# knight46/Quantum_compute_DFT

Hardware: AMD Instinct MI355X
Metric: grid_points_per_sec (higher is better)
Workload: dtype f64; 1 GPU; benzene_gga_def2svp: DFT_ComputeXC (GGA) nao=114 ngrid=143556 per GPU, synthetic AO/grid (SURVEY 8(d) recipe), inputs resident in HBM; functional=GGA, nao=114, nocc=21, ngrid_per_gpu=143556, entry_point=DFT_ComputeXC (the reference ABI: full density matrix)

## Files before the change

### include/dft_solver.h

```cpp
#ifndef QCDFT_AMD_DFT_SOLVER_H
#define QCDFT_AMD_DFT_SOLVER_H

#ifdef __cplusplus
extern "C" {
#endif

typedef struct XCSolver XCSolver;

enum SolverType { SOLVER_LDA = 0, SOLVER_GGA = 1, SOLVER_B3LYP = 2,
                  SOLVER_MIX = 3  };

enum XCComponent { XC_SLATER_X = 0, XC_VWN5_C, XC_VWN_RPA_C, XC_PW92_C,
                   XC_PBE_X, XC_PBE_C, XC_B88_X, XC_LYP_C, XC_NCOMP };


XCSolver *DFT_CreateSolver(int type);

void DFT_DestroySolver(XCSolver *solver);

double DFT_ComputeXC(XCSolver *solver, int ngrid, int nao,
                     unsigned long long d_dm_ptr,
                     unsigned long long d_ao_ptr,
                     unsigned long long d_ao_grad_ptr,
                     unsigned long long d_weights_ptr,
// ... 149 lines not shown
int DFT_ComputeXCGradient(XCSolver *solver, long long ngrid, int nao, unsigned long long d_dm_ptr,
                          unsigned long long d_ao_ptr, unsigned long long d_weights_ptr, unsigned long long d_ao_grad_ptr,
                          unsigned long long d_ao_hess_ptr, unsigned long long d_out_ptr);
int DFT_ComputeXCGradientSpin(XCSolver *solver, long long ngrid, int nao, unsigned long long d_dm_a_ptr,
                              unsigned long long d_dm_b_ptr, unsigned long long d_ao_ptr, unsigned long long d_weights_ptr,
                              unsigned long long d_ao_grad_ptr, unsigned long long d_ao_hess_ptr,
                              unsigned long long d_out_ptr);

int DFT_ComputeXCGradientMeta(XCSolver *solver, long long ngrid, int nao, unsigned long long d_dm_ptr,
                              unsigned long long d_ao_ptr, unsigned long long d_weights_ptr,
                              unsigned long long d_ao_grad_ptr, unsigned long long d_ao_hess_ptr,
                              unsigned long long d_out_ptr);
int DFT_ComputeXCEnergyDensityMeta(XCSolver *solver, long long ngrid, int nao, unsigned long long d_dm_ptr,
                                   unsigned long long d_ao_ptr, unsigned long long d_ao_grad_ptr,
                                   unsigned long long d_e_out_ptr);

int DFT_ComputeXCEnergyDensity(XCSolver *solver, long long ngrid, int nao, unsigned long long d_dm_ptr,
                               unsigned long long d_ao_ptr, unsigned long long d_ao_grad_ptr, unsigned long long d_e_out_ptr);
int DFT_ComputeXCEnergyDensitySpin(XCSolver *solver, long long ngrid, int nao, unsigned long long d_dm_a_ptr,
                                   unsigned long long d_dm_b_ptr, unsigned long long d_ao_ptr, unsigned long long d_ao_grad_ptr,
                                   unsigned long long d_e_out_ptr);
int DFT_BeckeWeightGradient(XCSolver *solver, long long ngrid, int natm, const double *atom_xyz, const double *atom_radius,
                            unsigned long long d_coords_ptr, unsigned long long d_owner_ptr, unsigned long long d_f_ptr,
                            unsigned long long d_cell_out_ptr, unsigned long long d_out_ptr);

void *DFT_EriColumnsOpen(int nshell, const double *shl_xyz, const int *shl_l, const int *shl_nprim,
                         const int *shl_off, const int *shl_ao, const double *prim_exp, const double *prim_coef,
                         int nao, int nprim_total, const double *qmax_pairs);
int DFT_EriColumns(void *handle, int shell_C, int shell_D, double screen, unsigned long long d_out_ptr);
int DFT_EriColumnsMany(void *handle, int npairs, const int *shell_C, const int *shell_D, double screen,
                       unsigned long long d_out_ptr, const long long *offsets);
int DFT_EriColumnsSetStream(void *handle, unsigned long long hip_stream);
const char *DFT_EriColumnsLastError(void *handle);
void DFT_EriColumnsClose(void *handle);

void *DFT_PointCoulombOpen(int nshell, const double *shl_xyz, const int *shl_l, const int *shl_nprim,
                           const int *shl_off, const int *shl_ao, const double *prim_exp, const double *prim_coef,
                           int nao, int nprim_total);
int DFT_PointCoulombMatrix(void *handle, long long npts, unsigned long long d_points_xyz, unsigned long long d_weights,
                           unsigned long long d_out);
int DFT_PointCoulombContract(void *handle, long long npts, unsigned long long d_points_xyz, unsigned long long d_dm,
                             unsigned long long d_out);
int DFT_PointCoulombField(void *handle, long long npts, unsigned long long d_points_xyz, unsigned long long d_dm,
                          unsigned long long d_out);
int DFT_PointCoulombSetStream(void *handle, unsigned long long hip_stream);
const char *DFT_PointCoulombLastError(void *handle);
void DFT_PointCoulombClose(void *handle);

void *DFT_Grad2eOpen(int nshell, const double *shl_xyz, const int *shl_l, const int *shl_nprim, const int *shl_off,
                     const int *shl_ao, const double *prim_exp, const double *prim_coef, int nao, int nprim_total);
int DFT_Grad2e(void *handle, unsigned long long d_dm, double c_hf, unsigned long long d_out);
int DFT_Grad2eSpin(void *handle, unsigned long long d_dm, unsigned long long d_ms, double c_hf, unsigned long long d_out);
int DFT_Grad2eSetStream(void *handle, unsigned long long hip_stream);
const char *DFT_Grad2eLastError(void *handle);
void DFT_Grad2eClose(void *handle);

void *DFT_ScfTailOpen(int nao, int nocc, unsigned long long d_hcore, unsigned long long d_overlap, unsigned long long d_basis,
                      unsigned long long d_fock_out, unsigned long long d_mo_energy);
int DFT_ScfTailSetStream(void *handle, unsigned long long hip_stream);
int DFT_ScfTailStep(void *handle, int rotate, double c_hf, double tol, double canon_tol, int max_inner, int slot, int nhist,
                    const int *hist, const double *coef, unsigned long long d_J, unsigned long long d_K,
                    unsigned long long d_vraw, unsigned long long d_dm, unsigned long long d_cocc, unsigned long long d_exc);
int DFT_ScfTailFinish(void *handle, double c_hf, unsigned long long d_J, unsigned long long d_K, unsigned long long d_dm,
                      unsigned long long d_cocc);
int DFT_ScfTailMore(void *handle, int nsteps, unsigned long long d_J, unsigned long long d_K, unsigned long long d_dm,
                    unsigned long long d_cocc, unsigned long long d_exc);
int DFT_ScfTailSetStepsHint(void *handle, int nsteps);
int DFT_ScfTailWait(void *handle, double *out8);
int DFT_ScfTailGram(void *handle, double *host_out64);
int DFT_ScfTailStamps(void *handle, long long *host_out16);
const char *DFT_ScfTailLastError(void *handle);
void DFT_ScfTailClose(void *handle);

int DFT_SetOption(XCSolver *solver, const char *key, double value);

double DFT_GetOption(XCSolver *solver, const char *key);

int DFT_SetStream(XCSolver *solver, unsigned long long hip_stream);

const char *DFT_GetLastError(XCSolver *solver);

int DFT_GetTimings(XCSolver *solver, double *ms, const char **names, int max_entries);

#ifdef __cplusplus
}
#endif
#endif
```

### quantum_compute_dft_amd/csrc/dft_api.hip

```cpp
#include <hip/hip_runtime.h>

#include <cmath>
#include <cstdarg>
#include <cstdio>
#include <cstdint>
#include <cstdlib>
#include <cstring>
#include <algorithm>
#include <limits>
#include <string>
#include <type_traits>
#include <vector>

#include "../../include/dft_solver.h"
#include "ao_kernels.hpp"
#include "jk_kernels.hpp"
#include "cd_kernels.hpp"
#include "cd_response_kernels.hpp"
#include "xc_big_kernels.hpp"
#include "xc_ws_kernels.hpp"
#include "xc_kernels.hpp"
#include "xc_occ_launch.hpp"
#include "xc_tiny_launch.hpp"
#include "dm_factor_launch.hpp"
// ... 2302 lines not shown
    }
    if (!strcmp(key, "eri_symmetric")) { s->eri_sym = value == 2.0 ? 2 : value != 0.0; return 0; }
    if (!strcmp(key, "graph")) { s->graph = value > 0.0 ? 1 : value < 0.0 ? -1 : 0; return 0; }
    if (!strcmp(key, "quirks")) { s->quirks = value != 0.0; s->fxc[0].ngrid = 0; return 0; }
    if (!strcmp(key, "path")) { s->path = (int)value; return 0; }
    if (!strcmp(key, "profile")) { s->profile = value != 0.0; return 0; }
    if (!strcmp(key, "spin_wait")) { s->spin_wait = value != 0.0; return 0; }
    if (!strcmp(key, "strict_sync")) { s->strict_sync = value != 0.0; return 0; }
    if (!strcmp(key, "fuse_finish")) { s->fuse_finish = value != 0.0; return 0; }
    if (!strcmp(key, "vxc_fringe")) { s->vxc_fringe = value > 0.0 ? 1 : value < 0.0 ? -1 : 0; return 0; }
    if (!strcmp(key, "publish")) { s->publish = value > 0.0 ? 1 : value < 0.0 ? -1 : 0; return 0; }
    if (!strcmp(key, "sweep_order")) { s->sweep_order = (int)value & 3; return 0; }
    if (!strcmp(key, "occ")) { s->occ = value == 1.0 ? 1 : value == 2.0 ? 2 : 0; return 0; }
    if (!strcmp(key, "dm_factor")) { s->dm_factor = value != 0.0; return 0; }
    if (!strcmp(key, "tiny")) { s->tiny = value > 0.0 ? 1 : value < 0.0 ? -1 : 0; return 0; }
    if (!strcmp(key, "ao_pt")) { s->ao_pt = value == 16.0 ? 16 : value == 8.0 ? 8 : 0; return 0; }
    if (!strcmp(key, "ksplit")) { s->ksplit = value > 0 ? (int)value : 0; return 0; }
    if (!strcmp(key, "xcg_spin_fused")) { s->xcg_spin_fused = value != 0.0; return 0; }
    if (!strcmp(key, "meta_fused")) { s->meta_fused = value != 0.0; return 0; }
    if (!strcmp(key, "xcg_meta_fused")) { s->xcg_meta_fused = value != 0.0; return 0; }
    if (!strcmp(key, "tau_spin_fused")) { s->tau_spin_fused = value != 0.0; return 0; }
    return -1;
}

double DFT_GetOption(XCSolver *s, const char *key)
{
    const double unknown = std::numeric_limits<double>::quiet_NaN();
    if (!s || !key) return unknown;
    if (!strcmp(key, "publish")) return s->publish;
    if (!strcmp(key, "publish_probe")) return s->publish_ok ? 1.0 : 0.0;
    if (!strcmp(key, "publish_live")) return s->publish > 0 && s->publish_ok ? 1.0 : 0.0;
    if (!strcmp(key, "used_publish")) return s->used_publish;
    if (!strcmp(key, "vxc_fringe")) return s->vxc_fringe;
    if (!strcmp(key, "used_vxc_fringe")) return s->used_vxc_fringe;
    if (!strcmp(key, "fuse_finish")) return s->fuse_finish;
    if (!strcmp(key, "strict_sync")) return s->strict_sync;
    if (!strcmp(key, "spin_wait")) return s->spin_wait;
    if (!strcmp(key, "graph")) return s->graph;
    if (!strcmp(key, "tiny")) return s->tiny;
    if (!strcmp(key, "sweep_order")) return s->sweep_order;
    if (!strcmp(key, "path")) return s->path;
    if (!strcmp(key, "quirks")) return s->quirks;
    if (!strcmp(key, "occ")) return s->occ;
    if (!strcmp(key, "used_occ")) return s->used_occ;
    if (!strcmp(key, "dm_factor")) return s->dm_factor;
    if (!strcmp(key, "used_dm_factor")) return s->used_dm_factor;
    if (!strcmp(key, "xcg_spin_fused")) return s->xcg_spin_fused;
    if (!strcmp(key, "meta_fused")) return s->meta_fused;
    if (!strcmp(key, "xcg_meta_fused")) return s->xcg_meta_fused;
    if (!strcmp(key, "tau_spin_fused")) return s->tau_spin_fused;
    if (!strcmp(key, "dm_factor_rank")) return s->dm_factor_rank;
    return unknown;
}

int DFT_SetStream(XCSolver *s, unsigned long long hip_stream)
{
    if (!s) return -1;
    DeviceGuard dg(s);
    if (s->device_ok) (void)hipStreamSynchronize(s->stream);
    s->stream = (hipStream_t)hip_stream;
    return 0;
}

const char *DFT_GetLastError(XCSolver *s)
{
    return s ? s->last_error.c_str() : "";
}

int DFT_GetTimings(XCSolver *s, double *ms, const char **names, int max_entries)
{
    if (!s || !s->device_ok) return 0;
    DeviceGuard dg(s);
    (void)hipStreamSynchronize(s->stream);
    int n = 0;
    for (size_t i = 0; i < s->n_timed && n < max_entries; ++i, ++n) {
        float t = 0.f;
        if (hipEventElapsedTime(&t, s->timings[i].t0, s->timings[i].t1) != hipSuccess) t = -1.f;
        if (ms) ms[n] = t;
        if (names) names[n] = s->timings[i].name;
    }
    return n;
}

}
```

### quantum_compute_dft_amd/csrc/xc_ws_kernels.hpp

```cpp
#pragma once
#include <hip/hip_runtime.h>
#include "xc_kernels.hpp"

namespace qcdft {

#ifdef QCDFT_STAMPS
__device__ unsigned long long g_stamps[256 * 8 * 4];
#define QCDFT_T(var) unsigned long long var = __builtin_amdgcn_s_memtime()
#define QCDFT_ACC(slot, a, b) st_acc[slot] += (b) - (a)
#else
#define QCDFT_T(var)
#define QCDFT_ACC(slot, a, b)
#endif

constexpr int WS_ROWS = 16;
constexpr int WS_THREADS = 512;
constexpr int WS_RING = 4;
constexpr int WS_OT = 16;

template <int NT> struct WsCfg {
    static constexpr int NCOL = 16 * NT;
    static constexpr int JN = (NT + 1) / 2;
    static constexpr int LDA = NCOL + 2;
    static constexpr int LDX = ((NCOL + 31) / 32) * 32 + 16;
};

__device__ __forceinline__ unsigned ws_tile(unsigned ntile, unsigned b, unsigned s, unsigned nwg, int rev)
{
    const unsigned t = b + s * nwg;
    return rev ? ntile - 1u - t : t;
}

template <int NT, int FP>
__device__ __forceinline__ void vxc_ws_mfma_fringe(const double *Ps, const double *Qs, int tid, int wave, int nao, long nstep,
                                                   double *__restrict__ slab)
{
    using C = WsCfg<NT>;
    constexpr int NF = NT - 1, F0 = 16 * NF;
    constexpr int TILE = WS_ROWS * C::LDX;
    constexpr int NOPP = F0 + 4 > 64 ? 2 : 1;
    static_assert(NT >= 2 && F0 + 4 <= 128, "one whole tile at least, two opposite indices per lane at most");
    const int lane = tid & 63, li = lane & 15, lk = lane >> 4;
    constexpr bool FRW = FP > 0;
    constexpr int ROWS = FRW ? (NF > 6 ? 1 : 0) : 2, RA = ROWS ? ROWS : 1, NL = FRW ? 2 * FP : 1;
    const int nr = FRW || NF >= 6 ? ROWS : min(2, max(0, NF - 2 * wave));
    d4 acc[RA][NF];
#pragma unroll
    for (int i = 0; i < RA; ++i)
#pragma unroll
        for (int j = 0; j < NF; ++j) acc[i][j] = (d4){0.0, 0.0, 0.0, 0.0};
    double fa[NL][NOPP], fb[NL][NOPP];
#pragma unroll
    for (int f = 0; f < NL; ++f)
#pragma unroll
        for (int j = 0; j < NOPP; ++j) { fa[f][j] = 0.0; fb[f][j] = 0.0; }
    int opp[NOPP];
#pragma unroll
    for (int j = 0; j < NOPP; ++j) opp[j] = min(lane + 64 * j, C::NCOL - 1);

    const int fo = lk * C::LDX + li;
    double af[RA], bf[NF];
    auto load_frags = [&](int slot, int ks, double (&a_)[RA], double (&b_)[NF]) {
        if (ROWS == 0) return;
        const double *P = Ps + slot * TILE + fo + 4 * ks * C::LDX;
        const double *Q = Qs + slot * TILE + fo + 4 * ks * C::LDX;
#pragma unroll
        for (int i = 0; i < RA; ++i) a_[i] = Q[16 * min(2 * wave + i, NF - 1)];
#pragma unroll
        for (int j = 0; j < NF; ++j) b_[j] = P[16 * j];
    };
    auto fringe_pair = [&](const double *Pr, const double *Qr, const double (&po)[NOPP], const double (&qo)[NOPP], int f) {
        const double2 pf = *reinterpret_cast<const double2 *>(&Pr[F0 + f]);
        const double2 qf = *reinterpret_cast<const double2 *>(&Qr[F0 + f]);
#pragma unroll
        for (int j = 0; j < NOPP; ++j) {
            fa[f][j] += qf.x * po[j];
            fa[f + 1][j] += qf.y * po[j];
            fb[f][j] += qo[j] * pf.x;
            fb[f + 1][j] += qo[j] * pf.y;
        }
    };
#pragma unroll
    for (int i = 0; i < RA; ++i) af[i] = 0.0;
#pragma unroll
    for (int j = 0; j < NF; ++j) bf[j] = 0.0;
    for (long base = 0; base < nstep; base += WS_RING) {
#pragma unroll
        for (int u = 0; u < WS_RING; ++u) {
            const long step = base + u;
            if (step >= 2 && step < nstep) {
                if (step == 2) load_frags((u + 2) % WS_RING, 0, af, bf);
#pragma unroll
                for (int ks = 0; ks < WS_ROWS / 4; ++ks) {
                    double an[RA], bn[NF];
                    if (ks + 1 < WS_ROWS / 4) load_frags((u + 2) % WS_RING, ks + 1, an, bn);
                    else                      load_frags((u + 3) % WS_RING, 0, an, bn);
#pragma unroll
                    for (int i = 0; i < ROWS; ++i)
                        if (i < nr) {
#pragma unroll
                            for (int j = 0; j < NF; ++j) acc[i][j] = mfma_f64(af[i], bf[j], acc[i][j]);
                        }
                    if (FRW) {
#pragma unroll
                        for (int kk = 0; kk < 4; ++kk) {
                            const double *Pr = Ps + ((u + 2) % WS_RING) * TILE + (4 * ks + kk) * C::LDX;
                            const double *Qr = Qs + ((u + 2) % WS_RING) * TILE + (4 * ks + kk) * C::LDX;
                            double po[NOPP], qo[NOPP];
#pragma unroll
                            for (int j = 0; j < NOPP; ++j) { po[j] = Pr[opp[j]]; qo[j] = Qr[opp[j]]; }
                            fringe_pair(Pr, Qr, po, qo, 0);
                            if (FP > 1) fringe_pair(Pr, Qr, po, qo, 2);
                        }
                    }
#pragma unroll
                    for (int i = 0; i < RA; ++i) af[i] = an[i];
#pragma unroll
                    for (int j = 0; j < NF; ++j) bf[j] = bn[j];
                    __builtin_amdgcn_sched_barrier(0);
                }
            }
            __syncthreads();
        }
    }
#pragma unroll
    for (int i = 0; i < ROWS; ++i) {
        if (i >= nr) continue;
#pragma unroll
        for (int j = 0; j < NF; ++j)
#pragma unroll
            for (int r = 0; r < 4; ++r)
                slab[(size_t)(16 * (2 * wave + i) + lk + 4 * r) * nao + 16 * j + li] = acc[i][j][r];
    }
    if (FRW) {
#pragma unroll
        for (int f = 0; f < NL; ++f) {
            if (F0 + f >= nao) continue;
#pragma unroll
            for (int j = 0; j < NOPP; ++j) {
                const int o = lane + 64 * j;
                if (o < nao) slab[(size_t)(F0 + f) * nao + o] = fa[f][j];
                if (o < F0)  slab[(size_t)o * nao + F0 + f] = fb[f][j];
            }
        }
    }
}

template <int NT, bool GRAD, bool VEC, bool SYM, bool FR = false>
__global__ __launch_bounds__(WS_THREADS, 2) void k_vxc_ws(long ngrid, int nao,
                                                          const double *__restrict__ ao,
                                                          const double *__restrict__ gx,
                                                          const double *__restrict__ gy,
                                                          const double *__restrict__ gz,
                                                          const double *__restrict__ coef,
                                                          double *__restrict__ slabs, int rev)
{
    using C = WsCfg<NT>;
    constexpr int TILE = WS_ROWS * C::LDX;
    constexpr int NTW = (NT + 1) / 2;
    __shared__ double ring[2 * WS_RING * TILE];
    double *const Ps = ring, *const Qs = ring + WS_RING * TILE;

    const int tid = threadIdx.x;
    const int wave = __builtin_amdgcn_readfirstlane(tid >> 6);
    const long ntile = (ngrid + WS_ROWS - 1) / WS_ROWS;
    const long nloc = (ntile > (long)blockIdx.x) ? (ntile - blockIdx.x + gridDim.x - 1) / gridDim.x : 0;
    const long nstep = nloc + 2;

    if constexpr (FR) {
        static_assert(!FR || !SYM, "the fringe variant writes one-sided slabs");
        double *slab = slabs + (size_t)blockIdx.x * nao * nao;
        if (wave < 3)                                 vxc_ws_mfma_fringe<NT, 0>(Ps, Qs, tid, wave, nao, nstep, slab);
        else if (wave == 3 && nao - 16 * (NT - 1) <= 2) vxc_ws_mfma_fringe<NT, 1>(Ps, Qs, tid, 3, nao, nstep, slab);
        else if (wave == 3)                           vxc_ws_mfma_fringe<NT, 2>(Ps, Qs, tid, 3, nao, nstep, slab);
    }
    if (!FR && wave < 4) {
        const int lane = tid & 63, li = lane & 15, lk = lane >> 4;
        const int wa = wave >> 1, wb = wave & 1;
        const int na = (NT - wa + 1) / 2, nb = (NT - wb + 1) / 2;
        d4 acc[NTW][NTW];
#pragma unroll
        for (int i = 0; i < NTW; ++i)
#pragma unroll
            for (int j = 0; j < NTW; ++j) acc[i][j] = (d4){0.0, 0.0, 0.0, 0.0};

#ifdef QCDFT_STAMPS
        unsigned long long st_acc[4] = {0, 0, 0, 0};
#endif
        const int fo = lk * C::LDX + li;
        double af[NTW], bf[NTW];
        auto load_frags = [&](int slot, int ks, double (&a_)[NTW], double (&b_)[NTW]) {
            const double *P = Ps + slot * TILE + fo + 4 * ks * C::LDX;
            const double *Q = Qs + slot * TILE + fo + 4 * ks * C::LDX;
#pragma unroll
            for (int i = 0; i < NTW; ++i) {
                a_[i] = Q[16 * min(wa + 2 * i, NT - 1)];
                b_[i] = P[16 * min(wb + 2 * i, NT - 1)];
            }
        };
#pragma unroll
        for (int i = 0; i < NTW; ++i) { af[i] = 0.0; bf[i] = 0.0; }
        for (long base = 0; base < nstep; base += WS_RING) {
#pragma unroll
            for (int u = 0; u < WS_RING; ++u) {
                const long step = base + u;
                QCDFT_T(ta);
                if (step >= 2 && step < nstep) {
                    if (step == 2) load_frags((u + 2) % WS_RING, 0, af, bf);
#pragma unroll
                    for (int ks = 0; ks < WS_ROWS / 4; ++ks) {
                        double an[NTW], bn[NTW];
                        if (ks + 1 < WS_ROWS / 4) load_frags((u + 2) % WS_RING, ks + 1, an, bn);
                        else                      load_frags((u + 3) % WS_RING, 0, an, bn);
#pragma unroll
                        for (int i = 0; i < NTW; ++i)
#pragma unroll
                            for (int j = 0; j < NTW; ++j)
                                if ((2 * i + 1 < NT || i < na) && (2 * j + 1 < NT || j < nb))
                                    acc[i][j] = mfma_f64(af[i], bf[j], acc[i][j]);
#pragma unroll
                        for (int i = 0; i < NTW; ++i) { af[i] = an[i]; bf[i] = bn[i]; }
                    }
                }
                QCDFT_T(tb);
                __syncthreads();
                QCDFT_T(tc);
                QCDFT_ACC(0, ta, tb);
                QCDFT_ACC(1, tb, tc);
            }
        }
#ifdef QCDFT_STAMPS
        if ((tid & 63) == 0) { g_stamps[(blockIdx.x * 8 + wave) * 4 + 0] = st_acc[0]; g_stamps[(blockIdx.x * 8 + wave) * 4 + 1] = st_acc[1]; }
#endif
        double *slab = slabs + (size_t)blockIdx.x * nao * nao;
        if (!SYM) {
#pragma unroll
            for (int i = 0; i < NTW; ++i)
#pragma unroll
                for (int j = 0; j < NTW; ++j) {
                    if (i >= na || j >= nb) continue;
                    const int b = 16 * (wb + 2 * j) + li;
#pragma unroll
                    for (int r = 0; r < 4; ++r) {
                        const int a = 16 * (wa + 2 * i) + lk + 4 * r;
                        if (a < nao && b < nao) slab[(size_t)a * nao + b] = acc[i][j][r];
                    }
                }
        } else {
            constexpr int LDM = C::NCOL + 1;
            static_assert(LDM * C::NCOL <= 2 * WS_RING * TILE, "M tile must fit in the ring");
            double *M = ring;
#pragma unroll
            for (int i = 0; i < NTW; ++i)
#pragma unroll
                for (int j = 0; j < NTW; ++j) {
                    if (i >= na || j >= nb) continue;
                    const int b = 16 * (wb + 2 * j) + li;
#pragma unroll
                    for (int r = 0; r < 4; ++r) M[(16 * (wa + 2 * i) + lk + 4 * r) * LDM + b] = acc[i][j][r];
                }
        }
    } else if (wave >= 4) {
        __builtin_amdgcn_s_setprio(3);
        const int lt = tid - 256, row = lt >> 4, seg = lt & 15;
        const double *c0 = coef, *c1 = coef + (size_t)ngrid, *c2 = coef + 2 * (size_t)ngrid,
                     *c3 = coef + 3 * (size_t)ngrid;
        double p0[2][2 * C::JN], p1[2][2 * C::JN], p2[2][2 * C::JN], p3[2][2 * C::JN];
        double k0[2], k1[2], k2[2], k3[2];

        const long plane = ngrid * (long)nao;
        const unsigned voff = (unsigned)(row * nao + 2 * seg) * 8u, koff = (unsigned)row * 8u;
        const unsigned tile_b = (unsigned)(WS_ROWS * nao) * 8u, ktile_b = WS_ROWS * 8u;
        const unsigned plane_b = (unsigned)(plane * 8), coef_b = (unsigned)(ngrid * 8);
        const __amdgpu_buffer_rsrc_t r0 = plane_rsrc(ao, plane), r1 = plane_rsrc(GRAD ? gx : ao, plane),
                                     r2 = plane_rsrc(GRAD ? gy : ao, plane), r3 = plane_rsrc(GRAD ? gz : ao, plane),
                                     q0 = plane_rsrc(c0, ngrid), q1 = plane_rsrc(GRAD ? c1 : c0, ngrid),
                                     q2 = plane_rsrc(GRAD ? c2 : c0, ngrid), q3 = plane_rsrc(GRAD ? c3 : c0, ngrid);
        auto issue = [&](int set, unsigned s) {
            const bool live = s < (unsigned)nloc;
            const unsigned t = ws_tile((unsigned)ntile, blockIdx.x, s, gridDim.x, rev);
            const unsigned so = live ? t * tile_b : plane_b, ko = live ? t * ktile_b : coef_b;
            k0[set] = buf_load_f64(q0, koff, ko);
            if (GRAD) {
                k1[set] = buf_load_f64(q1, koff, ko);
                k2[set] = buf_load_f64(q2, koff, ko);
                k3[set] = buf_load_f64(q3, koff, ko);
            }
            buf_load_row<C::JN, VEC>(r0, voff, so, p0[set]);
            if (GRAD) {
                buf_load_row<C::JN, VEC>(r1, voff, so, p1[set]);
                buf_load_row<C::JN, VEC>(r2, voff, so, p2[set]);
                buf_load_row<C::JN, VEC>(r3, voff, so, p3[set]);
            }
        };
        issue(0, 0);
        __builtin_amdgcn_sched_barrier(0);
        issue(1, 1);
        __builtin_amdgcn_sched_barrier(0);
#ifdef QCDFT_STAMPS
        unsigned long long st_acc[4] = {0, 0, 0, 0};
#endif

        for (long base = 0; base < nstep; base += WS_RING) {
#pragma unroll
            for (int u = 0; u < WS_RING; ++u) {
                const long step = base + u;
                const int set = u & 1;
                QCDFT_T(ta);
#ifdef QCDFT_STAMPS
                asm volatile("s_waitcnt vmcnt(20)" ::: "memory");
#endif
                QCDFT_T(tw);
                {
                    double *P = Ps + u * TILE, *Q = Qs + u * TILE;
#pragma unroll
                    for (int j = 0; j < C::JN; ++j) {
                        const int c = 32 * j + 2 * seg;
                        if (c < C::NCOL) {
                            const double a0 = p0[set][2 * j], b0 = p0[set][2 * j + 1];
                            double qa = k0[set] * a0, qb = k0[set] * b0;
                            if (GRAD) {
                                qa += k1[set] * p1[set][2 * j] + k2[set] * p2[set][2 * j] + k3[set] * p3[set][2 * j];
                                qb += k1[set] * p1[set][2 * j + 1] + k2[set] * p2[set][2 * j + 1] + k3[set] * p3[set][2 * j + 1];
                            }
                            *reinterpret_cast<double2 *>(&Q[row * C::LDX + c]) = make_double2(qa, qb);
                            *reinterpret_cast<double2 *>(&P[row * C::LDX + c]) = make_double2(a0, b0);
                        }
                    }
                    QCDFT_T(tm);
                    issue(set, (unsigned)step + 2u);
                    QCDFT_ACC(3, tw, tm);
                }
                QCDFT_T(tb);
                __syncthreads();
                QCDFT_T(tc);
                QCDFT_ACC(0, ta, tw);
                QCDFT_ACC(1, tw, tb);
                QCDFT_ACC(2, tb, tc);
            }
        }
#ifdef QCDFT_STAMPS
        if ((tid & 63) == 0) { for (int q = 0; q < 4; ++q) g_stamps[(blockIdx.x * 8 + wave) * 4 + q] = st_acc[q]; }
#endif
    }
    if (SYM) {
        constexpr int LDM = C::NCOL + 1;
        const double *M = ring;
        __syncthreads();
        double *slab = slabs + (size_t)blockIdx.x * nao * nao;
        for (int e = tid; e < nao * nao; e += WS_THREADS) {
            const int a = e / nao, b = e - a * nao;
            slab[e] = M[a * LDM + b] + M[b * LDM + a];
        }
    }
}

template <int NT, bool GRAD, bool VEC>
__global__ __launch_bounds__(WS_THREADS, 2) void k_rho_ws(long ngrid, int nao,
                                                          const double *__restrict__ ao,
                                                          const double *__restrict__ gx,
                                                          const double *__restrict__ gy,
                                                          const double *__restrict__ gz,
                                                          const double *__restrict__ dm,
                                                          double *__restrict__ rho,
                                                          double *__restrict__ grad,
                                                          double *__restrict__ sigma, int rev)
{
    using C = WsCfg<NT>;
    constexpr int NKS = 4 * NT;
    constexpr int NTW = (NT + 3) / 4;
    constexpr int ATILE = WS_ROWS * C::LDA, XTILE = WS_ROWS * C::LDX;
    constexpr int NQ = GRAD ? 4 : 1;
    constexpr int LDS_ = WS_ROWS + 2, SQ = 320, STILE = NQ * SQ;
    static_assert(WS_ROWS * LDS_ <= SQ, "a partial-sum plane must fit its stride");
    __shared__ double As[WS_RING * ATILE];
    __shared__ double Xs[2 * XTILE];
    __shared__ double Ss[2 * STILE];
    __shared__ double Ob[(WS_OT + 1) * WS_ROWS * 4];

    const int tid = threadIdx.x;
    const int wave = __builtin_amdgcn_readfirstlane(tid >> 6);
    const unsigned ntile = (unsigned)((ngrid + WS_ROWS - 1) / WS_ROWS);
    const unsigned nwg = gridDim.x, wg = blockIdx.x;
    const unsigned nloc = ntile > wg ? (ntile - wg + nwg - 1) / nwg : 0u;
    const unsigned nstep = nloc + 3;

    if (wave < 4) {
        const int lane = tid & 63, li = lane & 15, lk = lane >> 4;
        const int nks = (nao + 3) >> 2;
        const bool two = NTW > 1 && wave + 4 < NT;
        double dreg[NTW][NKS];
#pragma unroll
        for (int i = 0; i < NTW; ++i) {
            const int tcol = min(wave + 4 * i, NT - 1);
            const int n = 16 * tcol + li;
#pragma unroll
            for (int ks = 0; ks < NKS; ++ks) {
                const int k = 4 * ks + lk;
                const bool in = k < nao && n < nao;
                const int kc = in ? k : 0, nc = in ? n : 0;
                const double v = 0.5 * (dm[(size_t)kc * nao + nc] + dm[(size_t)nc * nao + kc]);
                dreg[i][ks] = in ? v : 0.0;
            }
        }
        const double *sp = Ss + min(wave, NQ - 1) * SQ + li * LDS_ + lk;
        const double ones = wave == 0 ? 1.0 : 2.0;
        double *op = Ob + lk * 4 + wave;
        unsigned oslot = 0;
        for (unsigned base = 0; base < nstep; base += WS_RING) {
#pragma unroll
            for (int u = 0; u < WS_RING; ++u) {
                const unsigned step = base + u;
                if (step >= 1 && step <= nloc && wave < NT) {
                    const double *ap = As + ((u + 3) % WS_RING) * ATILE + li * C::LDA + lk;
                    double *X = Xs + ((u + 1) & 1) * XTILE;
                    d4 acc[NTW];
#pragma unroll
                    for (int i = 0; i < NTW; ++i) acc[i] = (d4){0.0, 0.0, 0.0, 0.0};
#pragma unroll
                    for (int ks = 0; ks < NKS; ++ks) {
                        if (ks < NKS - 3 || ks < nks) {
                            const double a = ap[4 * ks];
                            acc[0] = mfma_f64(a, dreg[0][ks], acc[0]);
                            if (NTW > 1) {
                                if (two) acc[NTW - 1] = mfma_f64(a, dreg[NTW - 1][ks], acc[NTW - 1]);
                            }
                        }
                    }
#pragma unroll
                    for (int r = 0; r < 4; ++r) {
                        X[(lk + 4 * r) * C::LDX + 16 * wave + li] = acc[0][r];
                        if (NTW > 1) {
                            if (two) X[(lk + 4 * r) * C::LDX + 16 * (wave + 4) + li] = acc[NTW - 1][r];
                        }
                    }
                }
                if (step >= 3 && step - 3 < nloc && wave < NQ) {
                    const double *S = sp + ((u + 1) & 1) * STILE;
                    d4 t = (d4){0.0, 0.0, 0.0, 0.0};
#pragma unroll
                    for (int ks = 0; ks < WS_ROWS / 4; ++ks) t = mfma_f64(S[4 * ks], ones, t);
                    if (li == 0) {
                        double *o = op + oslot * (WS_ROWS * 4);
#pragma unroll
                        for (int r = 0; r < 4; ++r) o[16 * r] = t[r];
                    }
                    oslot = oslot == WS_OT ? 0u : oslot + 1u;
                }
                __syncthreads();
            }
        }
    } else {
        __builtin_amdgcn_s_setprio(3);
        const int lt = tid - 256, row = lt >> 4, seg = lt & 15;
        double ph[2][2 * C::JN];
        double pgx[2][2 * C::JN], pgy[2][2 * C::JN], pgz[2][2 * C::JN];

        const long plane = ngrid * (long)nao;
        const unsigned voff = (unsigned)(row * nao + 2 * seg) * 8u;
        const unsigned tile_b = (unsigned)(WS_ROWS * nao) * 8u, plane_b = (unsigned)(plane * 8);
        const __amdgpu_buffer_rsrc_t r0 = plane_rsrc(ao, plane), r1 = plane_rsrc(GRAD ? gx : ao, plane),
                                     r2 = plane_rsrc(GRAD ? gy : ao, plane), r3 = plane_rsrc(GRAD ? gz : ao, plane);
        unsigned o_run = (rev ? ntile - 1u - wg : wg) * tile_b, left = nloc;
        const unsigned o_inc = rev ? 0u - nwg * tile_b : nwg * tile_b;
        auto next_off = [&]() {
            const unsigned o = left ? o_run : plane_b;
            left = left ? left - 1u : 0u;
            o_run += o_inc;
            return o;
        };
        auto issue_ao = [&](int set, unsigned so) { buf_load_row<C::JN, VEC>(r0, voff, so, ph[set]); };
        auto issue_grad = [&](int set, unsigned so) {
            buf_load_row<C::JN, VEC>(r1, voff, so, pgx[set]);
            buf_load_row<C::JN, VEC>(r2, voff, so, pgy[set]);
            buf_load_row<C::JN, VEC>(r3, voff, so, pgz[set]);
        };
        unsigned o_a = next_off(), o_b = next_off();
        issue_ao(0, o_a);
        __builtin_amdgcn_sched_barrier(0);
        if (GRAD) issue_grad(0, plane_b);
        __builtin_amdgcn_sched_barrier(0);
        issue_ao(1, o_b);
        __builtin_amdgcn_sched_barrier(0);
        if (GRAD) issue_grad(1, plane_b);
        __builtin_amdgcn_sched_barrier(0);

        auto flush = [&](unsigned j0, unsigned slot0) {
            const unsigned j = j0 + (unsigned)(lt >> 4);
            const int r = lt & 15;
            if (j < nloc) {
                const long g = (long)ws_tile(ntile, wg, j, nwg, rev) * WS_ROWS + r;
                if (g < ngrid) {
                    unsigned slot = slot0 + (unsigned)(lt >> 4);
                    slot = slot > (unsigned)WS_OT ? slot - (WS_OT + 1) : slot;
                    const double *o = Ob + (slot * WS_ROWS + r) * 4;
                    rho[g] = o[0];
                    if (GRAD) {
                        const double ax = o[1], ay = o[2], az = o[3];
                        grad[3 * g + 0] = ax;
                        grad[3 * g + 1] = ay;
                        grad[3 * g + 2] = az;
                        sigma[g] = ax * ax + ay * ay + az * az;
                    }
                }
            }
        };
        unsigned flushed = 0, fslot = 0, fcount = WS_OT + 3 + 1;
        double *const sw = Ss + row * LDS_ + seg;
        for (unsigned base = 0; base < nstep; base += WS_RING) {
#pragma unroll
            for (int u = 0; u < WS_RING; ++u) {
                const int set = u & 1;
                const unsigned o_c = next_off();
                {
                    double *A = As + u * ATILE;
#pragma unroll
                    for (int j = 0; j < C::JN; ++j) {
                        const int c = 32 * j + 2 * seg;
                        if (c < C::NCOL)
                            *reinterpret_cast<double2 *>(&A[row * C::LDA + c]) = make_double2(ph[set][2 * j], ph[set][2 * j + 1]);
                    }
                    issue_ao(set, o_c);
                }
                {
                    const double *A = As + ((u + 2) % WS_RING) * ATILE;
                    const double *X = Xs + (u & 1) * XTILE;
                    double s0 = 0.0, s1 = 0.0, s2 = 0.0, s3 = 0.0;
#pragma unroll
                    for (int j = 0; j < C::JN; ++j) {
                        const int c = 32 * j + 2 * seg;
                        if (c < C::NCOL) {
                            const double2 x = *reinterpret_cast<const double2 *>(&X[row * C::LDX + c]);
                            const double2 p = *reinterpret_cast<const double2 *>(&A[row * C::LDA + c]);
                            const double t0 = x.x * p.x + x.y * p.y;
                            const double t1 = x.x * pgx[set][2 * j] + x.y * pgx[set][2 * j + 1];
                            const double t2 = x.x * pgy[set][2 * j] + x.y * pgy[set][2 * j + 1];
                            const double t3 = x.x * pgz[set][2 * j] + x.y * pgz[set][2 * j + 1];
                            if (j == 0) {
                                s0 = t0;
                                if (GRAD) { s1 = t1; s2 = t2; s3 = t3; }
                            } else {
                                s0 += t0;
                                if (GRAD) { s1 += t1; s2 += t2; s3 += t3; }
                            }
                        }
                    }
                    double *S = sw + (u & 1) * STILE;
                    S[0] = s0;
                    if (GRAD) { S[SQ] = s1; S[2 * SQ] = s2; S[3 * SQ] = s3; }
                }
                if (--fcount == 0) {
                    flush(flushed, fslot);
                    flushed += WS_OT;
                    fslot = fslot == 0 ? (unsigned)WS_OT : fslot - 1u;
                    fcount = WS_OT;
                }
                if (GRAD) issue_grad(set, o_a);
                o_a = o_b;
                o_b = o_c;
                __syncthreads();
            }
        }
        flush(flushed, fslot);
    }
}

__global__ __launch_bounds__(256) void k_finish_exc(long npart, const double *__restrict__ partial,
                                                    double *__restrict__ exc_dev, double *exc_host)
{
    __shared__ double part[4];
    double x = 0.0;
    for (long i = threadIdx.x; i < npart; i += 256) x += partial[i];
    for (int m = 32; m >= 1; m >>= 1) x += __shfl_down(x, m, 64);
    if ((threadIdx.x & 63) == 0) part[threadIdx.x >> 6] = x;
    __syncthreads();
    if (threadIdx.x == 0) {
        const double e = (part[0] + part[1]) + (part[2] + part[3]);
        exc_dev[0] = e;
        if (exc_host) {
            *(volatile double *)exc_host = e;
            __threadfence_system();
        }
    }
}

__global__ void k_publish_exc(const double *__restrict__ exc_dev, double *exc_host)
{
    *(volatile double *)exc_host = exc_dev[0];
    __threadfence_system();
}

template <bool SYM, bool FIN = false>
__global__ __launch_bounds__(256) void k_reduce_slabs8(int nao, int nslab,
                                                       const double *__restrict__ slabs,
                                                       double *__restrict__ V,
                                                       long npart = 0, const double *__restrict__ partial = nullptr,
                                                       double *__restrict__ exc_dev = nullptr, double *exc_host = nullptr)
{
    __shared__ double part[256];
    const size_t n2 = (size_t)nao * nao;
    const int el = threadIdx.x & 31, grp = threadIdx.x >> 5;
    const size_t e = (size_t)blockIdx.x * 32 + el;
    double s = 0.0;
    if (e < n2) {
        const int a = (int)(e / nao), b = (int)(e - (size_t)a * nao);
        const size_t et = (size_t)b * nao + a;
        int k = grp;
        for (; k + 8 * 15 < nslab; k += 8 * 16) {
            double v[16];
#pragma unroll
            for (int q = 0; q < 16; ++q) {
                v[q] = slabs[(size_t)(k + 8 * q) * n2 + e];
                if (SYM) v[q] += slabs[(size_t)(k + 8 * q) * n2 + et];
            }
#pragma unroll
            for (int q = 0; q < 16; ++q) s += v[q];
        }
        for (; k < nslab; k += 8) {
            double v = slabs[(size_t)k * n2 + e];
            if (SYM) v += slabs[(size_t)k * n2 + et];
            s += v;
        }
    }
    part[threadIdx.x] = s;
    __syncthreads();
    if (grp == 0 && e < n2) {
        const double *p = &part[el];
        V[e] = ((p[0] + p[32]) + (p[64] + p[96])) + ((p[128] + p[160]) + (p[192] + p[224]));
    }
    if (FIN) {
        if (blockIdx.x == gridDim.x - 1) {
            __syncthreads();
            double x = 0.0;
            for (long i = threadIdx.x; i < npart; i += 256) x += partial[i];
            part[threadIdx.x] = x;
            __syncthreads();
            for (int m = 128; m >= 1; m >>= 1) {
                if ((int)threadIdx.x < m) part[threadIdx.x] += part[threadIdx.x + m];
                __syncthreads();
            }
            if (threadIdx.x == 0) {
                exc_dev[0] = part[0];
                if (exc_host) {
                    *(volatile double *)exc_host = part[0];
                    __threadfence_system();
// ... 32 lines not shown
```

Measured before the change: 656.4 million grid-points/s.

## Deal Vxc MFMA output tiles to waves via a static per-size tile map

```diff
diff --git a/include/dft_solver.h b/include/dft_solver.h
--- a/include/dft_solver.h
+++ b/include/dft_solver.h
@@ -255,6 +255,8 @@
 
 int DFT_GetTimings(XCSolver *solver, double *ms, const char **names, int max_entries);
 
+int DFT_GetVxcDeal(int n, int fringe_form, int wave, int *rows, int *cols, int max_tiles, int *fringe_side);
+
 #ifdef __cplusplus
 }
 #endif
diff --git a/quantum_compute_dft_amd/csrc/dft_api.hip b/quantum_compute_dft_amd/csrc/dft_api.hip
--- a/quantum_compute_dft_amd/csrc/dft_api.hip
+++ b/quantum_compute_dft_amd/csrc/dft_api.hip
@@ -2408,4 +2408,16 @@
     return n;
 }
 
-}
+int DFT_GetVxcDeal(int n, int fringe_form, int wave, int *rows, int *cols, int max_tiles, int *fringe_side)
+{
+    if (n < 1 || n > (fringe_form ? 7 : 8) || wave < 0 || wave > 3) return -1;
+    if (fringe_side) *fringe_side = fringe_form ? vxc_fringe_side(wave) : 0;
+    const VxcShare s = vxc_share(n, wave);
+    for (int t = 0; t < s.ntile && t < max_tiles; ++t) {
+        if (rows) rows[t] = s.row[s.ti[t]];
+        if (cols) cols[t] = s.col[s.tj[t]];
+    }
+    return s.ntile;
+}
+
+}
diff --git a/quantum_compute_dft_amd/csrc/xc_ws_kernels.hpp b/quantum_compute_dft_amd/csrc/xc_ws_kernels.hpp
--- a/quantum_compute_dft_amd/csrc/xc_ws_kernels.hpp
+++ b/quantum_compute_dft_amd/csrc/xc_ws_kernels.hpp
@@ -1,5 +1,6 @@
 #pragma once
 #include <hip/hip_runtime.h>
+#include <type_traits>
 #include "xc_kernels.hpp"
 
 namespace qcdft {
@@ -8,9 +9,13 @@
 __device__ unsigned long long g_stamps[256 * 8 * 4];
 #define QCDFT_T(var) unsigned long long var = __builtin_amdgcn_s_memtime()
 #define QCDFT_ACC(slot, a, b) st_acc[slot] += (b) - (a)
+#define QCDFT_MARK(slot) do { if ((threadIdx.x & 63) == 0) g_stamps[(blockIdx.x * 8 + (threadIdx.x >> 6)) * 4 + (slot)] = __builtin_amdgcn_s_memtime(); } while (0)
+#define QCDFT_DRAIN() asm volatile("s_waitcnt vmcnt(0)" ::: "memory")
 #else
 #define QCDFT_T(var)
 #define QCDFT_ACC(slot, a, b)
+#define QCDFT_MARK(slot) do {} while (0)
+#define QCDFT_DRAIN() do {} while (0)
 #endif
 
 constexpr int WS_ROWS = 16;
@@ -31,24 +36,101 @@
     return rev ? ntile - 1u - t : t;
 }
 
-template <int NT, int FP>
-__device__ __forceinline__ void vxc_ws_mfma_fringe(const double *Ps, const double *Qs, int tid, int wave, int nao, long nstep,
-                                                   double *__restrict__ slab)
+constexpr char VXC_DEAL[8][8][9] = {
+    {"0"},
+    {"01",
+     "23"},
+    {"000",
+     "111",
+     "222"},
+    {"0011",
+     "0011",
+     "2233",
+     "2233"},
+    {"00011",
+     "00011",
+     "02111",
+     "22233",
+     "22233"},
+    {"000111",
+     "000111",
+     "000111",
+     "222333",
+     "222333",
+     "222333"},
+    {"0011122",
+     "0011122",
+     "0011122",
+     "0011222",
+     "0011222",
+     "0033333",
+     "0233333"},
+    {"00001111",
+     "00001111",
+     "00001111",
+     "00001111",
+     "22223333",
+     "22223333",
+     "22223333",
+     "22223333"},
+};
+
+struct VxcShare {
+    int ntile = 0, nrow = 0, ncol = 0;
+    int row[8] = {}, col[8] = {};
+    int ti[16] = {}, tj[16] = {};
+};
+
+constexpr VxcShare vxc_share(int n, int w)
+{
+    VxcShare s;
+    for (int r = 0; r < n; ++r)
+        for (int c = 0; c < n; ++c) {
+            if (VXC_DEAL[n - 1][r][c] - '0' != w) continue;
+            int i = 0, j = 0;
+            while (i < s.nrow && s.row[i] != r) ++i;
+            if (i == s.nrow) s.row[s.nrow++] = r;
+            while (j < s.ncol && s.col[j] != c) ++j;
+            if (j == s.ncol) s.col[s.ncol++] = c;
+            s.ti[s.ntile] = i;
+            s.tj[s.ntile] = j;
+            ++s.ntile;
+        }
+    return s;
+}
+
+template <int N, int W> struct VxcShareOf { static constexpr VxcShare v = vxc_share(N, W); };
+
+template <int I, int E, class F>
+__device__ __forceinline__ void ws_static_for(F &&f)
+{
+    if constexpr (I < E) {
+        f(std::integral_constant<int, I>{});
+        ws_static_for<I + 1, E>(f);
+    }
+}
+
+constexpr int vxc_fringe_side(int w) { return w == 3 ? 3 : 0; }
+
+template <int NT, bool SYM, bool FR, int W, int FP>
+__device__ __forceinline__ void vxc_ws_mfma_role(const double *Ps, const double *Qs, int tid, int nao, long nstep,
+                                                 double *__restrict__ out)
 {
     using C = WsCfg<NT>;
-    constexpr int NF = NT - 1, F0 = 16 * NF;
+    constexpr int N = FR ? NT - 1 : NT, F0 = 16 * N;
     constexpr int TILE = WS_ROWS * C::LDX;
-    constexpr int NOPP = F0 + 4 > 64 ? 2 : 1;
-    static_assert(NT >= 2 && F0 + 4 <= 128, "one whole tile at least, two opposite indices per lane at most");
+    using SH = VxcShareOf<N, W>;
+    constexpr VxcShare S = SH::v;
+    constexpr int NA = S.ntile ? S.ntile : 1, NR = S.nrow ? S.nrow : 1, NC = S.ncol ? S.ncol : 1;
+    constexpr int SIDE = FR && FP > 0 ? vxc_fringe_side(W) : 0;
+    constexpr int NL = FP > 0 ? 2 * FP : 1;
+    constexpr int NOPP = FR && F0 + 4 > 64 ? 2 : 1;
+    static_assert(!FR || (NT >= 2 && !SYM && F0 + 4 <= 128), "one whole tile at least, two opposite indices per lane at most; one-sided slabs");
+    static_assert(FR || FP == 0, "fringe lines belong to the FR form");
     const int lane = tid & 63, li = lane & 15, lk = lane >> 4;
-    constexpr bool FRW = FP > 0;
-    constexpr int ROWS = FRW ? (NF > 6 ? 1 : 0) : 2, RA = ROWS ? ROWS : 1, NL = FRW ? 2 * FP : 1;
-    const int nr = FRW || NF >= 6 ? ROWS : min(2, max(0, NF - 2 * wave));
-    d4 acc[RA][NF];
-#pragma unroll
-    for (int i = 0; i < RA; ++i)
-#pragma unroll
-        for (int j = 0; j < NF; ++j) acc[i][j] = (d4){0.0, 0.0, 0.0, 0.0};
+    d4 acc[NA];
+#pragma unroll
+    for (int t = 0; t < NA; ++t) acc[t] = (d4){0.0, 0.0, 0.0, 0.0};
     double fa[NL][NOPP], fb[NL][NOPP];
 #pragma unroll
     for (int f = 0; f < NL; ++f)
@@ -58,20 +140,20 @@
 #pragma unroll
     for (int j = 0; j < NOPP; ++j) opp[j] = min(lane + 64 * j, C::NCOL - 1);
 
+#ifdef QCDFT_STAMPS
+    unsigned long long st_acc[4] = {0, 0, 0, 0};
+#endif
     const int fo = lk * C::LDX + li;
-    double af[RA], bf[NF];
-    auto load_frags = [&](int slot, int ks, double (&a_)[RA], double (&b_)[NF]) {
-        if (ROWS == 0) return;
+    double af[NR], bf[NC];
+    auto load_frags = [&](int slot, int ks, double (&a_)[NR], double (&b_)[NC]) {
         const double *P = Ps + slot * TILE + fo + 4 * ks * C::LDX;
         const double *Q = Qs + slot * TILE + fo + 4 * ks * C::LDX;
-#pragma unroll
-        for (int i = 0; i < RA; ++i) a_[i] = Q[16 * min(2 * wave + i, NF - 1)];
-#pragma unroll
-        for (int j = 0; j < NF; ++j) b_[j] = P[16 * j];
+        ws_static_for<0, S.nrow>([&](auto ic) { constexpr int i = decltype(ic)::value; a_[i] = Q[16 * SH::v.row[i]]; });
+        ws_static_for<0, S.ncol>([&](auto jc) { constexpr int j = decltype(jc)::value; b_[j] = P[16 * SH::v.col[j]]; });
     };
-    auto fringe_pair = [&](const double *Pr, const double *Qr, const double (&po)[NOPP], const double (&qo)[NOPP], int f) {
-        const double2 pf = *reinterpret_cast<const double2 *>(&Pr[F0 + f]);
-        const double2 qf = *reinterpret_cast<const double2 *>(&Qr[F0 + f]);
+    auto fringe_pair = [&](const double *pr, const double *qr, const double (&po)[NOPP], const double (&qo)[NOPP], int f) {
+        const double2 pf = *reinterpret_cast<const double2 *>(&pr[f]);
+        const double2 qf = *reinterpret_cast<const double2 *>(&qr[f]);
 #pragma unroll
         for (int j = 0; j < NOPP; ++j) {
             fa[f][j] += qf.x * po[j];
@@ -81,66 +163,91 @@
         }
     };
 #pragma unroll
-    for (int i = 0; i < RA; ++i) af[i] = 0.0;
-#pragma unroll
-    for (int j = 0; j < NF; ++j) bf[j] = 0.0;
+    for (int i = 0; i < NR; ++i) af[i] = 0.0;
+#pragma unroll
+    for (int j = 0; j < NC; ++j) bf[j] = 0.0;
     for (long base = 0; base < nstep; base += WS_RING) {
 #pragma unroll
         for (int u = 0; u < WS_RING; ++u) {
             const long step = base + u;
+            QCDFT_T(ta);
             if (step >= 2 && step < nstep) {
                 if (step == 2) load_frags((u + 2) % WS_RING, 0, af, bf);
+                int xp = ((u + 2) % WS_RING) * TILE + F0, xq = xp + WS_RING * TILE, yp[NOPP], yq[NOPP];
+#pragma unroll
+                for (int j = 0; j < NOPP; ++j) { yp[j] = ((u + 2) % WS_RING) * TILE + opp[j]; yq[j] = yp[j] + WS_RING * TILE; }
+                if (SIDE) {
+                    asm volatile("" : "+v"(xp), "+v"(xq));
+#pragma unroll
+                    for (int j = 0; j < NOPP; ++j) asm volatile("" : "+v"(yp[j]), "+v"(yq[j]));
+                }
 #pragma unroll
                 for (int ks = 0; ks < WS_ROWS / 4; ++ks) {
-                    double an[RA], bn[NF];
+                    double an[NR], bn[NC];
                     if (ks + 1 < WS_ROWS / 4) load_frags((u + 2) % WS_RING, ks + 1, an, bn);
                     else                      load_frags((u + 3) % WS_RING, 0, an, bn);
-#pragma unroll
-                    for (int i = 0; i < ROWS; ++i)
-                        if (i < nr) {
-#pragma unroll
-                            for (int j = 0; j < NF; ++j) acc[i][j] = mfma_f64(af[i], bf[j], acc[i][j]);
+                    ws_static_for<0, 4>([&](auto kc) {
+                        constexpr int kk = decltype(kc)::value;
+                        if (SIDE) {
+                            const int ro = (4 * ks + kk) * C::LDX;
+                            double po[NOPP], qo[NOPP];
+#pragma unroll
+                            for (int j = 0; j < NOPP; ++j) { po[j] = Ps[yp[j] + ro]; qo[j] = Ps[yq[j] + ro]; }
+                            fringe_pair(Ps + xp + ro, Ps + xq + ro, po, qo, 0);
+                            if (FP > 1) fringe_pair(Ps + xp + ro, Ps + xq + ro, po, qo, 2);
                         }
-                    if (FRW) {
-#pragma unroll
-                        for (int kk = 0; kk < 4; ++kk) {
-                            const double *Pr = Ps + ((u + 2) % WS_RING) * TILE + (4 * ks + kk) * C::LDX;
-                            const double *Qr = Qs + ((u + 2) % WS_RING) * TILE + (4 * ks + kk) * C::LDX;
-                            double po[NOPP], qo[NOPP];
-#pragma unroll
-                            for (int j = 0; j < NOPP; ++j) { po[j] = Pr[opp[j]]; qo[j] = Qr[opp[j]]; }
-                            fringe_pair(Pr, Qr, po, qo, 0);
-                            if (FP > 1) fringe_pair(Pr, Qr, po, qo, 2);
-                        }
+                        ws_static_for<kk * S.ntile / 4, (kk + 1) * S.ntile / 4>([&](auto tc) {
+                            constexpr int t = decltype(tc)::value;
+                            acc[t] = mfma_f64(af[SH::v.ti[t]], bf[SH::v.tj[t]], acc[t]);
+                        });
+                    });
+#pragma unroll
+                    for (int i = 0; i < NR; ++i) af[i] = an[i];
+#pragma unroll
+                    for (int j = 0; j < NC; ++j) bf[j] = bn[j];
+                    if (SIDE) {
+                        __builtin_amdgcn_sched_group_barrier(0x100, 64, 0);
+                        ws_static_for<0, 4>([&](auto kc) {
+                            constexpr int kk = decltype(kc)::value;
+                            constexpr int nm = (kk + 1) * S.ntile / 4 - kk * S.ntile / 4;
+                            if (nm) __builtin_amdgcn_sched_group_barrier(0x008, nm, 0);
+                            __builtin_amdgcn_sched_group_barrier(0x002, 4 * FP * NOPP, 0);
+                        });
                     }
-#pragma unroll
-                    for (int i = 0; i < RA; ++i) af[i] = an[i];
-#pragma unroll
-                    for (int j = 0; j < NF; ++j) bf[j] = bn[j];
-                    __builtin_amdgcn_sched_barrier(0);
-                }
-            }
+                    if (FR) __builtin_amdgcn_sched_barrier(0);
+                }
+            }
+            QCDFT_T(tb);
             __syncthreads();
-        }
-    }
-#pragma unroll
-    for (int i = 0; i < ROWS; ++i) {
-        if (i >= nr) continue;
-#pragma unroll
-        for (int j = 0; j < NF; ++j)
-#pragma unroll
-            for (int r = 0; r < 4; ++r)
-                slab[(size_t)(16 * (2 * wave + i) + lk + 4 * r) * nao + 16 * j + li] = acc[i][j][r];
-    }
-    if (FRW) {
+            QCDFT_T(tc);
+            QCDFT_ACC(0, ta, tb);
+            QCDFT_ACC(1, tb, tc);
+        }
+    }
+#ifdef QCDFT_STAMPS
+    if ((tid & 63) == 0) { g_stamps[(blockIdx.x * 8 + W) * 4 + 0] = st_acc[0]; g_stamps[(blockIdx.x * 8 + W) * 4 + 1] = st_acc[1]; }
+#endif
+    constexpr int LDM = C::NCOL + 1;
+    ws_static_for<0, S.ntile>([&](auto tc) {
+        constexpr int t = decltype(tc)::value;
+        const int b = 16 * SH::v.col[SH::v.tj[t]] + li;
+#pragma unroll
+        for (int r = 0; r < 4; ++r) {
+            const int a = 16 * SH::v.row[SH::v.ti[t]] + lk + 4 * r;
+            if (SYM)                          out[a * LDM + b] = acc[t][r];
+            else if (FR)                      out[(size_t)a * nao + b] = acc[t][r];
+            else if (a < nao && b < nao)      out[(size_t)a * nao + b] = acc[t][r];
+        }
+    });
+    if (SIDE) {
 #pragma unroll
         for (int f = 0; f < NL; ++f) {
             if (F0 + f >= nao) continue;
 #pragma unroll
             for (int j = 0; j < NOPP; ++j) {
                 const int o = lane + 64 * j;
-                if (o < nao) slab[(size_t)(F0 + f) * nao + o] = fa[f][j];
-                if (o < F0)  slab[(size_t)o * nao + F0 + f] = fb[f][j];
+                if (o < nao) out[(size_t)(F0 + f) * nao + o] = fa[f][j];
+                if (o < F0)  out[(size_t)o * nao + F0 + f] = fb[f][j];
             }
         }
     }
@@ -157,7 +264,6 @@
 {
     using C = WsCfg<NT>;
     constexpr int TILE = WS_ROWS * C::LDX;
-    constexpr int NTW = (NT + 1) / 2;
     __shared__ double ring[2 * WS_RING * TILE];
     double *const Ps = ring, *const Qs = ring + WS_RING * TILE;
 
@@ -167,100 +273,31 @@
     const long nloc = (ntile > (long)blockIdx.x) ? (ntile - blockIdx.x + gridDim.x - 1) / gridDim.x : 0;
     const long nstep = nloc + 2;
 
-    if constexpr (FR) {
+    if (wave < 4) {
         static_assert(!FR || !SYM, "the fringe variant writes one-sided slabs");
-        double *slab = slabs + (size_t)blockIdx.x * nao * nao;
-        if (wave < 3)                                 vxc_ws_mfma_fringe<NT, 0>(Ps, Qs, tid, wave, nao, nstep, slab);
-        else if (wave == 3 && nao - 16 * (NT - 1) <= 2) vxc_ws_mfma_fringe<NT, 1>(Ps, Qs, tid, 3, nao, nstep, slab);
-        else if (wave == 3)                           vxc_ws_mfma_fringe<NT, 2>(Ps, Qs, tid, 3, nao, nstep, slab);
-    }
-    if (!FR && wave < 4) {
-        const int lane = tid & 63, li = lane & 15, lk = lane >> 4;
-        const int wa = wave >> 1, wb = wave & 1;
-        const int na = (NT - wa + 1) / 2, nb = (NT - wb + 1) / 2;
-        d4 acc[NTW][NTW];
-#pragma unroll
-        for (int i = 0; i < NTW; ++i)
-#pragma unroll
-            for (int j = 0; j < NTW; ++j) acc[i][j] = (d4){0.0, 0.0, 0.0, 0.0};
-
-#ifdef QCDFT_STAMPS
-        unsigned long long st_acc[4] = {0, 0, 0, 0};
-#endif
-        const int fo = lk * C::LDX + li;
-        double af[NTW], bf[NTW];
-        auto load_frags = [&](int slot, int ks, double (&a_)[NTW], double (&b_)[NTW]) {
-            const double *P = Ps + slot * TILE + fo + 4 * ks * C::LDX;
-            const double *Q = Qs + slot * TILE + fo + 4 * ks * C::LDX;
-#pragma unroll
-            for (int i = 0; i < NTW; ++i) {
-                a_[i] = Q[16 * min(wa + 2 * i, NT - 1)];
-                b_[i] = P[16 * min(wb + 2 * i, NT - 1)];
-            }
-        };
-#pragma unroll
-        for (int i = 0; i < NTW; ++i) { af[i] = 0.0; bf[i] = 0.0; }
-        for (long base = 0; base < nstep; base += WS_RING) {
-#pragma unroll
-            for (int u = 0; u < WS_RING; ++u) {
-                const long step = base + u;
-                QCDFT_T(ta);
-                if (step >= 2 && step < nstep) {
-                    if (step == 2) load_frags((u + 2) % WS_RING, 0, af, bf);
-#pragma unroll
-                    for (int ks = 0; ks < WS_ROWS / 4; ++ks) {
-                        double an[NTW], bn[NTW];
-                        if (ks + 1 < WS_ROWS / 4) load_frags((u + 2) % WS_RING, ks + 1, an, bn);
-                        else                      load_frags((u + 3) % WS_RING, 0, an, bn);
-#pragma unroll
-                        for (int i = 0; i < NTW; ++i)
-#pragma unroll
-                            for (int j = 0; j < NTW; ++j)
-                                if ((2 * i + 1 < NT || i < na) && (2 * j + 1 < NT || j < nb))
-                                    acc[i][j] = mfma_f64(af[i], bf[j], acc[i][j]);
-#pragma unroll
-                        for (int i = 0; i < NTW; ++i) { af[i] = an[i]; bf[i] = bn[i]; }
-                    }
-                }
-                QCDFT_T(tb);
-                __syncthreads();
-                QCDFT_T(tc);
-                QCDFT_ACC(0, ta, tb);
-                QCDFT_ACC(1, tb, tc);
-            }
-        }
-#ifdef QCDFT_STAMPS
-        if ((tid & 63) == 0) { g_stamps[(blockIdx.x * 8 + wave) * 4 + 0] = st_acc[0]; g_stamps[(blockIdx.x * 8 + wave) * 4 + 1] = st_acc[1]; }
-#endif
-        double *slab = slabs + (size_t)blockIdx.x * nao * nao;
-        if (!SYM) {
-#pragma unroll
-            for (int i = 0; i < NTW; ++i)
-#pragma unroll
-                for (int j = 0; j < NTW; ++j) {
-                    if (i >= na || j >= nb) continue;
-                    const int b = 16 * (wb + 2 * j) + li;
-#pragma unroll
-                    for (int r = 0; r < 4; ++r) {
-                        const int a = 16 * (wa + 2 * i) + lk + 4 * r;
-                        if (a < nao && b < nao) slab[(size_t)a * nao + b] = acc[i][j][r];
-                    }
-                }
+        static_assert(!SYM || (C::NCOL + 1) * C::NCOL <= 2 * WS_RING * TILE, "M tile must fit in the ring");
+        double *out = SYM ? ring : slabs + (size_t)blockIdx.x * nao * nao;
+        if constexpr (FR) {
+            const bool two = nao - 16 * (NT - 1) > 2;
+            switch (wave) {
+            case 0:  vxc_ws_mfma_role<NT, false, true, 0, 0>(Ps, Qs, tid, nao, nstep, out); break;
+            case 1:  vxc_ws_mfma_role<NT, false, true, 1, 0>(Ps, Qs, tid, nao, nstep, out); break;
+            case 2:  vxc_ws_mfma_role<NT, false, true, 2, 0>(Ps, Qs, tid, nao, nstep, out); break;
+            default:
+                if (two) vxc_ws_mfma_role<NT, false, true, 3, 2>(Ps, Qs, tid, nao, nstep, out);
+                else     vxc_ws_mfma_role<NT, false, true, 3, 1>(Ps, Qs, tid, nao, nstep, out);
+                break;
+            }
         } else {
-            constexpr int LDM = C::NCOL + 1;
-            static_assert(LDM * C::NCOL <= 2 * WS_RING * TILE, "M tile must fit in the ring");
-            double *M = ring;
-#pragma unroll
-            for (int i = 0; i < NTW; ++i)
-#pragma unroll
-                for (int j = 0; j < NTW; ++j) {
-                    if (i >= na || j >= nb) continue;
-                    const int b = 16 * (wb + 2 * j) + li;
-#pragma unroll
-                    for (int r = 0; r < 4; ++r) M[(16 * (wa + 2 * i) + lk + 4 * r) * LDM + b] = acc[i][j][r];
-                }
-        }
-    } else if (wave >= 4) {
+            switch (wave) {
+            case 0:  vxc_ws_mfma_role<NT, SYM, false, 0, 0>(Ps, Qs, tid, nao, nstep, out); break;
+            case 1:  vxc_ws_mfma_role<NT, SYM, false, 1, 0>(Ps, Qs, tid, nao, nstep, out); break;
+            case 2:  vxc_ws_mfma_role<NT, SYM, false, 2, 0>(Ps, Qs, tid, nao, nstep, out); break;
+            default: vxc_ws_mfma_role<NT, SYM, false, 3, 0>(Ps, Qs, tid, nao, nstep, out); break;
+            }
+        }
+    }
+    if (wave >= 4) {
         __builtin_amdgcn_s_setprio(3);
         const int lt = tid - 256, row = lt >> 4, seg = lt & 15;
         const double *c0 = coef, *c1 = coef + (size_t)ngrid, *c2 = coef + 2 * (size_t)ngrid,
@@ -387,6 +424,7 @@
 
     if (wave < 4) {
         const int lane = tid & 63, li = lane & 15, lk = lane >> 4;
+        QCDFT_MARK(0);
         const int nks = (nao + 3) >> 2;
         const bool two = NTW > 1 && wave + 4 < NT;
         double dreg[NTW][NKS];
@@ -412,6 +450,7 @@
             for (int u = 0; u < WS_RING; ++u) {
                 const unsigned step = base + u;
                 if (step >= 1 && step <= nloc && wave < NT) {
+                    if (step == 1) { QCDFT_DRAIN(); QCDFT_MARK(1); }
                     const double *ap = As + ((u + 3) % WS_RING) * ATILE + li * C::LDA + lk;
                     double *X = Xs + ((u + 1) & 1) * XTILE;
                     d4 acc[NTW];
@@ -448,10 +487,13 @@
                     oslot = oslot == WS_OT ? 0u : oslot + 1u;
                 }
                 __syncthreads();
-            }
-        }
+                if (step == 0) QCDFT_MARK(2);
+            }
+        }
+        QCDFT_MARK(3);
     } else {
         __builtin_amdgcn_s_setprio(3);
+        QCDFT_MARK(0);
         const int lt = tid - 256, row = lt >> 4, seg = lt & 15;
         double ph[2][2 * C::JN];
         double pgx[2][2 * C::JN], pgy[2][2 * C::JN], pgz[2][2 * C::JN];
@@ -558,9 +600,12 @@
                 if (GRAD) issue_grad(set, o_a);
                 o_a = o_b;
                 o_b = o_c;
+                if (base + u == 0) QCDFT_MARK(1);
                 __syncthreads();
-            }
-        }
+                if (base + u == 0) QCDFT_MARK(2);
+            }
+        }
+        QCDFT_MARK(3);
         flush(flushed, fslot);
     }
 }
```

After: 659.1 million grid-points/s, median of 2. About the same (+0.4%).
